# phantomzone-org/fhe-ram

Hardware: AMD Instinct MI355X
Metric: encrypted RAM read ops/s + write ops/s at 2^18 entries; achieved HBM GB/s vs peak (higher is better)
Workload: dtype f64

## Files before the change

fhe-ram_amd/csrc/bank.hpp:

```cpp
#pragma once
#include "path.hpp"

struct fheram_bank {
    fheram_ctx* c = nullptr;
    int M = 0, mws = 0;
    RamState ram[FHERAM_BANK_MAX];
    double* d_prep = nullptr;
    double* d_prep_inv = nullptr;
    ReadBufs list;
    int list_n = 0;
};

namespace {

RamView bank_view(const fheram_bank* b, int first) {
    RamView v = ctx_view(b->c);
    const size_t o1 = (size_t)first * b->mws * fheram_ctx::GLWE, oR = o1 * b->c->rows;
    for (int32_t** p : {&v.rows, &v.A, &v.B, &v.C, &v.D}) *p += oR;
    for (int32_t** p : {&v.part, &v.tmp, &v.tmp2, &v.res, &v.tree, &v.w, &v.trtop}) *p += o1;
    return v;
}
Opnds bank_opnds(fheram_bank* b, RamState* st, const fheram_addr* const* addrs, int n) {
    if (n == 1) return one_addr(b->c, addrs, b->mws, st);
    return table_opnds(b->c, st, addrs, n, b->mws, b->d_prep, b->d_prep_inv, SRC_MAP_IDENTITY, true);
// ... 127 lines not shown
    return FHERAM_OK;
}
void fheram_bank_destroy(fheram_bank* b) {
    if (!b) return;
    if (b->c) {
        hipSetDevice(b->c->device);
        if (b->c->stream) hipStreamSynchronize(b->c->stream);
        if (b->c->stream2) hipStreamSynchronize(b->c->stream2);
    }
    if (b->d_prep) hipFree(b->d_prep);
    if (b->d_prep_inv) hipFree(b->d_prep_inv);
    reads_free(b->list);
    fheram_ctx_destroy(b->c);
    delete b;
}
const char* fheram_bank_last_error(const fheram_bank* b) { return fheram_last_error(b ? b->c : nullptr); }
int fheram_bank_size(const fheram_bank* b) { return b ? b->M : 0; }

int fheram_bank_keys_load(fheram_bank* b, const int64_t* gal_els, int n_gal, const int64_t* const* atk_glwe,
                          const int64_t* atk_ggsw_inv, int64_t atk_ggsw_inv_p, const int64_t* tsk) {
    if (!b) return FHERAM_ERR_INVALID_ARG;
    const int rc = fheram_keys_load(b->c, gal_els, n_gal, atk_glwe, atk_ggsw_inv, atk_ggsw_inv_p, tsk);
    if (rc != FHERAM_OK) return rc;
    for (int m = 0; m < b->M; m++) { b->ram[m].memo_top = false; b->ram[m].memo_alone = 0; }
    return FHERAM_OK;
}
int fheram_bank_ram_upload(fheram_bank* b, int member, const int64_t* rows) {
    if (!b) return FHERAM_ERR_INVALID_ARG;
    fheram_ctx* c = b->c;
    if (member < 0 || member >= b->M) return fail(c, FHERAM_ERR_INVALID_ARG, "no such member");
    if (!rows) return fail(c, FHERAM_ERR_INVALID_ARG, "null rows");
    HIPCHK(c, hipSetDevice(c->device));
    const size_t n = (size_t)b->mws * c->rows * fheram_ctx::GLWE;
    const int rc = upload_i64(c, c->d_data + (size_t)member * n, rows, n);
    if (rc != FHERAM_OK) return rc;
    RamState& r = b->ram[member];
    r.initialized = true; r.state = false; r.memo_top = false; r.memo_alone = 0;
    return FHERAM_OK;
}
int fheram_bank_ram_download(fheram_bank* b, int member, int64_t* rows) {
    if (!b) return FHERAM_ERR_INVALID_ARG;
    fheram_ctx* c = b->c;
    if (member < 0 || member >= b->M || !rows) return fail(c, FHERAM_ERR_INVALID_ARG, "no such member, or null rows");
    if (!b->ram[member].initialized) return fail(c, FHERAM_ERR_UNINITIALIZED, "unitialized memory: self.data.len()=0");
    HIPCHK(c, hipSetDevice(c->device));
    const size_t n = (size_t)b->mws * c->rows * fheram_ctx::GLWE;
    const int rc = download_i64(c, rows, c->d_data + (size_t)member * n, n);
    return rc == FHERAM_OK ? check_precision(c) : rc;
}
int fheram_bank_ram_tree_download(fheram_bank* b, int member, int level, int64_t* out) {
    if (!b) return FHERAM_ERR_INVALID_ARG;
    fheram_ctx* c = b->c;
    if (member < 0 || member >= b->M || !out) return fail(c, FHERAM_ERR_INVALID_ARG, "no such member, or null output");
    if (level != 0 || c->n2 < 2) return fail(c, FHERAM_ERR_INVALID_ARG, "tree level does not exist (ram.rs:315-324)");
    HIPCHK(c, hipSetDevice(c->device));
    const size_t n = (size_t)b->mws * fheram_ctx::GLWE;
    return download_i64(c, out, c->d_tree + (size_t)member * n, n);
}
int fheram_bank_ram_state(const fheram_bank* b, int member) { return (b && member >= 0 && member < b->M) ? (int)b->ram[member].state : 0; }

int fheram_bank_address_create(fheram_bank* b, const int64_t* const* ggsw, int n_ggsw, fheram_addr** out) {
    if (!b) return FHERAM_ERR_INVALID_ARG;
    return fheram_address_create(b->c, ggsw, n_ggsw, out);
}

int fheram_bank_fheuint_create(fheram_bank* b, const int64_t* bits, int n_bits, fheram_fheuint** out) {
// ... 104 lines not shown
```

fhe-ram_amd/csrc/ctx.hpp:

```cpp
#pragma once
#include "../../include/fheram.h"
#include "kernels.hpp"
#include "cmux_chain.hpp"

#include <algorithm>
#include <atomic>
#include <cstdio>
#include <cstdlib>
#include <cstring>
#include <map>
#include <string>
#include <vector>

using namespace fk;

namespace {

thread_local std::string g_create_err;


struct ProfCls {
    uint64_t launches = 0, blocks = 0;
    double ms = 0.0;
    std::vector<std::pair<hipEvent_t, hipEvent_t>> pending;
};

}

inline uint64_t next_addr_id() { static std::atomic<uint64_t> n{0}; return ++n; }

struct RamState {
    bool initialized = false, state = false;
    bool memo_top = false;
    int memo_alone = 0;
    bool res_in_trtop = false;
};

struct ReadBufs {
    int cap = 0;
    int32_t *A = nullptr, *B = nullptr;
    int32_t* C = nullptr;
    int32_t *res = nullptr, *tmp = nullptr, *tmp2 = nullptr;
    double* prep = nullptr;
    int64_t *h_res = nullptr, *d_h_res = nullptr;
};

struct fheram_ctx {
    fheram_params p;
    int device = 0;
    hipStream_t stream = nullptr;
    hipStream_t stream2 = nullptr;
    hipStream_t cur = nullptr;
    hipEvent_t ev_fork = nullptr, ev_join = nullptr;
    hipEvent_t ev_xout = nullptr, ev_xin = nullptr;
    bool side_begun = false;
    bool trhi_in_C = false;
    bool tree_rotate_pending = false;
    int ws = 0, n2 = 0, n_digits = 0;
    size_t rows = 0;
    size_t rows_glob = 0;
    int shard = 0, n_shards = 1;
    std::vector<std::vector<int>> base2d;
    static constexpr int S_CT = 3, S_ADDR = 4, S_INV = 5, DNUM_CT = 3, DNUM_GGSW = 4;
    int s_evk = 4;
    size_t atk = 0;
    static constexpr size_t GLWE = (size_t)S_CT * 2 * N;
    static constexpr size_t GLWE4 = (size_t)S_ADDR * 2 * N;
    static constexpr size_t GGSW = (size_t)DNUM_CT * 2 * GLWE4;
    static constexpr size_t EVK5 = (size_t)DNUM_GGSW * S_INV * 2 * N;
    static constexpr size_t GGSW5 = (size_t)DNUM_GGSW * 2 * S_INV * 2 * N;
    double* d_tw = nullptr;
    double ninv = 0.0;
    double* d_atk = nullptr;
    double* d_atk_inv = nullptr;
    double* d_tsk = nullptr;
    int64_t gal[LOGN];
    bool keys_loaded = false;
    int32_t* d_data = nullptr;
    int32_t* d_tree = nullptr;
    int32_t* d_scrA = nullptr;
    int32_t* d_scrB = nullptr;
    int32_t* d_scrC = nullptr;
    int32_t* d_scrD = nullptr;
    int32_t* d_res = nullptr;
    int32_t* d_tmp = nullptr;
    int32_t* d_tmp2 = nullptr;
    int32_t* d_w = nullptr;
    double* d_big = nullptr;
    double* d_big2 = nullptr;
    int limb_split = 1;
// ... 233 lines not shown
```

fhe-ram_amd/csrc/fheram.hip:

```cpp
#include <unistd.h>
#include <atomic>
#include "path.hpp"

extern "C" {

int fheram_params_default(fheram_params* p) {
    if (!p) return FHERAM_ERR_INVALID_ARG;
    std::memset(p, 0, sizeof(*p));
    p->log_n = 12; p->base2k = 17; p->rank = 1;
    p->k_glwe_pt = 3; p->k_glwe_ct = 51; p->k_ggsw_addr = 68; p->k_evk_trace = 68; p->k_evk_ggsw_inv = 85;
    p->word_size = 4; p->n_decomp = 4;
    p->decomp_n[0] = p->decomp_n[1] = p->decomp_n[2] = p->decomp_n[3] = 3;
    p->max_addr = (uint64_t)1 << 14;
    return FHERAM_OK;
}

const char* fheram_last_error(const fheram_ctx* c) { return c ? c->err.c_str() : g_create_err.c_str(); }

void fheram_config_default(fheram_config* cfg) {
    if (!cfg) return;
    fheram_config d{};
    d.limb_split = 1; d.fine_split = 1; d.memo = 1; d.pre_inv = 1; d.tail = 1; d.tail_test = 0; d.mid = 2; d.mid_test = 0;
    d.chain = 1; d.chain_y = 3; d.pair_z = 1; d.fuse = 1; d.graph = 0; d.safe = 0; d.nco = 0; d.tail_ep = 1; d.monitor = 1; d.reserved = 0;
    auto env = [](const char* n) { const char* v = getenv(n); return (v && v[0]) ? v[0] : '\0'; };
// ... 71 lines not shown
        while (bits != 0) {
            std::vector<int> v;
            for (uint32_t i = 0; i < p->n_decomp; i++) {
                const uint32_t b = p->decomp_n[i];
                if (b <= bits) { v.push_back((int)b); bits -= b; }
                else { if (bits != 0) { v.push_back((int)bits); bits = 0; } break; }
            }
            c->base2d.push_back(v);
        }
    }
    c->n2 = (int)c->base2d.size();
    for (auto& v : c->base2d) { c->n_digits += (int)v.size(); c->max_digits = std::max(c->max_digits, (int)v.size()); }
    for (int i = 0; i < LOGN; i++) c->gal[i] = galois_element(i);

#define CCHK(call)                                                                  \
    do {                                                                            \
        hipError_t e_ = (call);                                                     \
        if (e_ != hipSuccess) {                                                     \
            g_create_err = std::string(#call) + ": " + hipGetErrorString(e_);       \
            fheram_ctx_destroy(c);                                                  \
            return FHERAM_ERR_DEVICE;                                               \
        }                                                                           \
    } while (0)
    CCHK(hipSetDevice(device));
    CCHK(hipStreamCreateWithFlags(&c->stream, hipStreamNonBlocking));
    {
        int lo = 0, hi = 0;
        CCHK(hipDeviceGetStreamPriorityRange(&lo, &hi));
        CCHK(hipStreamCreateWithPriority(&c->stream2, hipStreamNonBlocking, lo));
    }
    c->cur = c->stream;
    CCHK(hipEventCreateWithFlags(&c->ev_fork, hipEventDisableTiming));
    CCHK(hipEventCreateWithFlags(&c->ev_join, hipEventDisableTiming));
    CCHK(hipEventCreateWithFlags(&c->ev_xout, hipEventDisableTiming));
    CCHK(hipEventCreateWithFlags(&c->ev_xin, hipEventDisableTiming));
    CCHK(hipEventCreate(&c->t0));
    CCHK(hipEventCreate(&c->t1));
    {
        fheram_config cfg;
        if (user_cfg) cfg = *user_cfg; else fheram_config_default(&cfg);
        c->limb_split = cfg.limb_split ? 1 : 0;
        c->fine_split = cfg.fine_split ? 1 : 0;
        c->memo = cfg.memo ? 1 : 0;
        c->pre_inv = c->memo ? (cfg.pre_inv == 2 ? 2 : (cfg.pre_inv ? 1 : 0)) : 0;
        c->tail = cfg.tail ? 1 : 0;
        static std::atomic<int> serial{0};
        c->tail_xoff = ((serial++ + (int)getpid()) & 1) * (TAIL_GROUPS / 2);
        c->tail_test = cfg.tail_test < 0 ? 0 : (cfg.tail_test > 2 ? 2 : cfg.tail_test);
        c->tail_ep = cfg.tail_ep ? 1 : 0;
        c->mid = cfg.mid < 0 ? 0 : (cfg.mid > 2 ? 2 : cfg.mid);
        c->mid_test = cfg.mid_test ? 1 : 0;
        c->chain = cfg.chain ? 1 : 0;
        c->chain_y = cfg.chain_y ? 3 : 0;
        c->pair_z = cfg.pair_z ? 1 : 0;
        c->fuse = cfg.fuse ? 1 : 0;
        c->use_graph = cfg.graph ? 1 : 0;
        if (c->use_graph) c->pre_inv = 0;
        c->safe = cfg.safe ? 1 : 0;
        if (c->safe) { c->tail = 0; c->tail_test = 0; c->mid = 0; c->mid_test = 0; if (c->pre_inv == 1) c->pre_inv = 2; }
        c->monitor = cfg.monitor < 0 ? 0 : (cfg.monitor > 2 ? 2 : cfg.monitor);
        if (c->safe && c->monitor == 1) c->monitor = 2;
        c->nco = cfg.nco == 2 ? 2 : (cfg.nco == 1 ? 1 : 0);
        hipDeviceProp_t prop;
        if (hipGetDeviceProperties(&prop, device) == hipSuccess && prop.multiProcessorCount > 0) c->cus = prop.multiProcessorCount;
    }
#define LDSATTR(k) CCHK(hipFuncSetAttribute(reinterpret_cast<const void*>(k), hipFuncAttributeMaxDynamicSharedMemorySize, (int)LDS_BYTES))
    LDSATTR(k_prepare);
    LDSATTR((&k_ext_product<3, 4, 1>));
    LDSATTR((&k_ext_product<3, 4, 2>));
    LDSATTR((&k_ext_product<3, 4, 1, 1>));
    LDSATTR((&k_ext_product_fine<3, 4>));
    LDSATTR((&k_ext_product_fine<4, 5>));
    LDSATTR((&k_ext_product_chain<3, 4>));
    LDSATTR((&k_ext_product_chain_r<4>));
    LDSATTR((&k_pair_z<4>)); LDSATTR((&k_pair_z<5>));
    LDSATTR((&k_read_chain<4, 4>)); LDSATTR((&k_read_chain<5, 4>)); LDSATTR((&k_write_chain<4, 4>)); LDSATTR((&k_write_chain<5, 4>));
    LDSATTR((&k_write_chain_t<4, 4>)); LDSATTR((&k_write_chain_t<5, 4>));
    LDSATTR((&k_read_chain_w<4, 4>)); LDSATTR((&k_read_chain_w<5, 4>));
    LDSATTR((&k_read_chain_t<4, 4>)); LDSATTR((&k_read_chain_t<5, 4>));
    LDSATTR((&k_trace_tail_t<3, 4, 3>)); LDSATTR((&k_trace_tail_t<3, 5, 3>));
    LDSATTR((&k_keyswitch_chain_w<3, 4, 3, 3>)); LDSATTR((&k_keyswitch_chain_w<3, 5, 3, 3>));
    LDSATTR((&k_keyswitch_chain<3, 4, 3>));
    LDSATTR((&k_keyswitch_chain<3, 4, 3, 3>));
    LDSATTR((&k_keyswitch_chain<3, 5, 3, 3>));
    LDSATTR((&k_trace_tail<3, 4, 3>));
    LDSATTR((&k_chain_mid<false, 4, 3, 2>)); LDSATTR((&k_chain_mid<false, 5, 3, 2>)); LDSATTR((&k_chain_mid<true, 4, 3, 2>));
    LDSATTR((&k_chain_mid<false, 4, 1, 1>)); LDSATTR((&k_chain_mid<false, 5, 1, 1>));
    LDSATTR((&k_chain_mid<false, 4, 1, 2>)); LDSATTR((&k_chain_mid<false, 5, 1, 2>));
#define LDSATTR_KS4(M, SX, SK, SO) LDSATTR((&k_keyswitch<M, SX, SK, SO, 1>)); LDSATTR((&k_keyswitch<M, SX, SK, SO, 1, 1>)); LDSATTR((&k_keyswitch_fine<M, SX, SK>))
#define LDSATTR_KS(M, SX, SK, SO) LDSATTR_KS4(M, SX, SK, SO); LDSATTR((&k_keyswitch<M, SX, SK, SO, 2>))
    LDSATTR_KS(KS_AUTO, 3, 4, 3);
    LDSATTR_KS(KS_TRACE, 3, 4, 3);
    LDSATTR_KS4(KS_PAIR, 3, 4, 3);
    LDSATTR_KS(KS_ADD, 3, 4, 3);
    LDSATTR_KS(KS_SUBNEG, 3, 4, 3);
// ... 54 lines not shown
    for (int i = 0; i < 2; i++) CCHK(hipEventCreateWithFlags(&c->ev_inv[i], hipEventDisableTiming));
    CCHK(hipEventCreateWithFlags(&c->ev_wdone, hipEventDisableTiming));
    CCHK(hipEventCreateWithFlags(&c->ev_opstart, hipEventDisableTiming));
    CCHK(hipMalloc(&c->d_tail_sync, (size_t)(TAIL_GROUPS + 1) * 32 * sizeof(unsigned)));
    CCHK(hipMemset(c->d_tail_sync, 0, (size_t)(TAIL_GROUPS + 1) * 32 * sizeof(unsigned)));
    for (int i = 0; i < 2; i++) {
        CCHK(hipMalloc(&c->d_mid_sync[i], (size_t)(MID_GROUPS_MAX + 1) * 32 * sizeof(unsigned)));
        CCHK(hipMemset(c->d_mid_sync[i], 0, (size_t)(MID_GROUPS_MAX + 1) * 32 * sizeof(unsigned)));
        CCHK(hipMalloc(&c->d_mid_y[i], (size_t)2 * MID_GROUPS_MAX * 2 * N * sizeof(double)));
        CCHK(hipMalloc(&c->d_mid_big[i], (size_t)2 * MID_GROUPS_MAX * BIG_STRIDE * sizeof(double)));
    }
    CCHK(hipHostMalloc((void**)&c->h_tail_fb, 64, hipHostMallocDefault));
    *c->h_tail_fb = 0;
    CCHK(hipHostMalloc((void**)&c->h_mid_fb, 128, hipHostMallocDefault));
    memset(c->h_mid_fb, 0, 128);
    CCHK(hipHostMalloc((void**)&c->h_res, ((size_t)c->ws * G + 1) * sizeof(int64_t), hipHostMallocMapped));
    CCHK(hipHostGetDevicePointer((void**)&c->d_h_res, c->h_res, 0));
    CCHK(hipHostMalloc((void**)&c->h_w, (size_t)c->ws * G * sizeof(int32_t), hipHostMallocDefault));
    CCHK(hipEventCreateWithFlags(&c->ev_w, hipEventDisableTiming));
#undef CCHK
    *out = c;
    return FHERAM_OK;
}

void fheram_ctx_destroy(fheram_ctx* c) {
    if (!c) return;
    hipSetDevice(c->device);
    if (c->stream) hipStreamSynchronize(c->stream);
    if (c->stream2) hipStreamSynchronize(c->stream2);
    prof_collect(c);
    reads_free(c->batch);
    if (c->ev_fork) hipEventDestroy(c->ev_fork);
    if (c->ev_join) hipEventDestroy(c->ev_join);
    for (int i = 0; i < 2; i++) if (c->ev_inv[i]) hipEventDestroy(c->ev_inv[i]);
    if (c->ev_wdone) hipEventDestroy(c->ev_wdone);
    if (c->ev_opstart) hipEventDestroy(c->ev_opstart);
    if (c->ev_xout) hipEventDestroy(c->ev_xout);
    if (c->ev_xin) hipEventDestroy(c->ev_xin);
    if (c->stream2) hipStreamDestroy(c->stream2);
    for (auto e : c->ev_pool) hipEventDestroy(e);
    if (c->t0) hipEventDestroy(c->t0);
    if (c->t1) hipEventDestroy(c->t1);
    for (int b = 0; b < 2; b++) { if (c->ev_pin[b]) hipEventDestroy(c->ev_pin[b]); if (c->h_pin[b]) hipHostFree(c->h_pin[b]); }
    void* bufs[] = {c->d_tw, c->d_atk, c->d_atk_inv, c->d_tsk, c->d_data, c->d_scrA, c->d_scrB, c->d_big, c->d_big2, c->d_scrC, c->d_scrD, c->d_ggsw_tmp2, c->d_tmp2, c->d_part, c->d_gat[0], c->d_gat[1], c->d_gat[2], c->d_tree, c->d_res, c->d_tmp, c->d_w, c->d_trtop, c->d_prep, c->d_ggsw_tmp, c->d_tail_sync, c->d_prep_inv, c->d_ggsw_inv, c->d_mid_sync[0], c->d_mid_sync[1], c->d_mid_y[0], c->d_mid_y[1], c->d_mid_big[0], c->d_mid_big[1]};
    for (void* b : bufs) if (b) hipFree(b);
    if (c->h_tail_fb) hipHostFree(c->h_tail_fb);
    if (c->h_mid_fb) hipHostFree(c->h_mid_fb);
    if (c->h_res) hipHostFree(c->h_res);
    if (c->h_ro_flag) hipHostFree(c->h_ro_flag);
    if (c->h_w) hipHostFree(c->h_w);
    if (c->ev_w) hipEventDestroy(c->ev_w);
    if (c->stream) hipStreamDestroy(c->stream);
    delete c;
}

int fheram_ctx_config(const fheram_ctx* c, fheram_config* out) {
    if (!c || !out) return FHERAM_ERR_INVALID_ARG;
    fheram_config d{};
    d.limb_split = c->limb_split; d.fine_split = c->fine_split; d.memo = c->memo; d.pre_inv = c->pre_inv; d.tail = c->tail; d.tail_test = c->tail_test;
    d.mid = c->mid; d.mid_test = c->mid_test; d.chain = c->chain; d.chain_y = c->chain_y; d.pair_z = c->pair_z; d.fuse = c->fuse;
    d.graph = c->use_graph; d.safe = c->safe; d.nco = c->nco; d.monitor = c->monitor; d.tail_ep = c->tail_ep;
    *out = d;
    return FHERAM_OK;
}

size_t fheram_glwe_len(const fheram_ctx*) { return fheram_ctx::GLWE; }
// ... 9 lines not shown
    if (!c) return FHERAM_ERR_INVALID_ARG;
    if (!gal_els || !atk_glwe || !atk_ggsw_inv || !tsk) return fail(c, FHERAM_ERR_INVALID_ARG, "null key pointer");
    if (n_gal != LOGN) return fail(c, FHERAM_ERR_KEYS, "expected log2(N) trace keys (keys.rs:39)");
    if (atk_ggsw_inv_p != -1) return fail(c, FHERAM_ERR_KEYS, "auto_key.p() != -1 (coordinate_prepared.rs:134)");
    HIPCHK(c, hipSetDevice(c->device));
    HIPCHK(c, hipStreamSynchronize(c->stream));
    HIPCHK(c, hipStreamSynchronize(c->stream2));
    int order[LOGN];
    for (int i = 0; i < LOGN; i++) {
        order[i] = -1;
        for (int j = 0; j < n_gal; j++) if (gal_els[j] == c->gal[i]) order[i] = j;
        if (order[i] < 0) return fail(c, FHERAM_ERR_KEYS, "missing trace key for a Galois element of GLWE::trace_galois_elements");
    }
    int32_t* d_stage = nullptr;
    const size_t stage_n = std::max(c->atk, fheram_ctx::EVK5);
    HIPCHK(c, hipMalloc(&d_stage, stage_n * sizeof(int32_t)));
    int rc = FHERAM_OK;
    for (int i = 0; i < LOGN && rc == FHERAM_OK; i++) {
        rc = upload_i64(c, d_stage, atk_glwe[order[i]], c->atk);
        if (rc == FHERAM_OK) launch_prepare(c, d_stage, c->d_atk + (size_t)i * c->atk, (int)(c->atk / N), c->gal[i]);
        hipStreamSynchronize(c->stream);
    }
    if (rc == FHERAM_OK) rc = upload_i64(c, d_stage, atk_ggsw_inv, fheram_ctx::EVK5);
    if (rc == FHERAM_OK) { launch_prepare(c, d_stage, c->d_atk_inv, (int)(fheram_ctx::EVK5 / N), -1); hipStreamSynchronize(c->stream); }
    if (rc == FHERAM_OK) rc = upload_i64(c, d_stage, tsk, fheram_ctx::EVK5);
    if (rc == FHERAM_OK) { launch_prepare(c, d_stage, c->d_tsk, (int)(fheram_ctx::EVK5 / N)); hipStreamSynchronize(c->stream); }
    hipFree(d_stage);
    if (rc != FHERAM_OK) return rc;
    HIPCHK(c, hipGetLastError());
    c->keys_loaded = true;
    c->inv_id[0] = c->inv_id[1] = 0;
    c->inv_pending[0] = c->inv_pending[1] = false;
    c->ram.memo_top = false; c->ram.memo_alone = 0;
    return FHERAM_OK;
}

int fheram_ram_upload(fheram_ctx* c, const int64_t* rows) {
    if (!c) return FHERAM_ERR_INVALID_ARG;
    if (!rows) return fail(c, FHERAM_ERR_INVALID_ARG, "null rows");
    HIPCHK(c, hipSetDevice(c->device));
    int rc = upload_i64(c, c->d_data, rows, (size_t)c->ws * c->rows * fheram_ctx::GLWE);
    if (rc != FHERAM_OK) return rc;
    c->ram.initialized = true; c->ram.state = false; c->ram.memo_top = false; c->ram.memo_alone = 0;
    return FHERAM_OK;
}
int fheram_ram_download(fheram_ctx* c, int64_t* rows) {
    if (!c || !rows) return FHERAM_ERR_INVALID_ARG;
    if (!c->ram.initialized) return fail(c, FHERAM_ERR_UNINITIALIZED, "unitialized memory: self.data.len()=0");
    HIPCHK(c, hipSetDevice(c->device));
    const int rc = download_i64(c, rows, c->d_data, (size_t)c->ws * c->rows * fheram_ctx::GLWE);
    return rc == FHERAM_OK ? check_precision(c) : rc;
}
int fheram_ram_tree_download(fheram_ctx* c, int level, int64_t* out) {
    if (!c || !out) return FHERAM_ERR_INVALID_ARG;
    if (level != 0 || c->n2 < 2) return fail(c, FHERAM_ERR_INVALID_ARG, "tree level does not exist (ram.rs:315-324)");
    HIPCHK(c, hipSetDevice(c->device));
    return download_i64(c, out, c->d_tree, (size_t)c->ws * fheram_ctx::GLWE);
}
int fheram_ram_state(const fheram_ctx* c) { return c ? (int)c->ram.state : 0; }

int fheram_address_create(fheram_ctx* c, const int64_t* const* ggsw, int n_ggsw, fheram_addr** out) {
    if (!c || !out) return FHERAM_ERR_INVALID_ARG;
    *out = nullptr;
    if (!ggsw) return fail(c, FHERAM_ERR_INVALID_ARG, "null ggsw");
    if (n_ggsw != c->n_digits) return fail(c, FHERAM_ERR_INVALID_ARG, "address digit count does not match the context's Base2D (ram.rs:404)");
    HIPCHK(c, hipSetDevice(c->device));
    fheram_addr* a = new fheram_addr{c, nullptr, n_ggsw, c->device};
    hipError_t e = hipMalloc(&a->d_ggsw, (size_t)n_ggsw * fheram_ctx::GGSW * sizeof(int32_t));
    if (e != hipSuccess) { delete a; return fail(c, FHERAM_ERR_DEVICE, std::string("hipMalloc: ") + hipGetErrorString(e)); }
    for (int i = 0; i < n_ggsw; i++) {
        if (!ggsw[i]) { fheram_address_destroy(a); return fail(c, FHERAM_ERR_INVALID_ARG, "null ggsw digit"); }
        int rc = upload_i64(c, a->d_ggsw + (size_t)i * fheram_ctx::GGSW, ggsw[i], fheram_ctx::GGSW);
        if (rc != FHERAM_OK) { fheram_address_destroy(a); return rc; }
// ... 498 lines not shown
```

fhe-ram_amd/csrc/path.hpp:

```cpp
#pragma once
#include "launch.hpp"

namespace {

struct Opnds {
    fheram_ctx* c;
    RamState* st;
    const fheram_addr* const* addrs;
    int n, ws;
    double *tab, *tab_inv;
    long stride;
    unsigned src_map;
    bool bank;
    int member(int k) const { return (int)((src_map >> (4 * k)) & 15u); }
    int Y() const { return n * ws; }
    double* prep(int k, int ci) const { return digits_of(c, tab + k * stride, ci); }
    double* inv(int k, int ci) const { return digits_of(c, tab_inv + k * stride, ci); }
    GlweRef slice(GlweRef r, int k) const { r.p += (long)k * ws * r.sy; return r; }
    GlweRef rows(GlweRef r, int k) const { return slice(r, member(k)); }
    OpndTable table() const { return n == 1 ? OpndTable{} : OpndTable{ws, stride, src_map}; }
    bool row_fuse(int d, int n_tr, int gx) const { return use_row_fuse(c, d, n_tr, gx, Y(), bank); }
};
Opnds one_addr(fheram_ctx* c, const fheram_addr* const* a, int ws, RamState* st) { return Opnds{c, st, a, 1, ws, c->d_prep, c->d_prep_inv, 0, 0, false}; }
Opnds one_addr(fheram_ctx* c, const fheram_addr* const* a) { return one_addr(c, a, c->ws, &c->ram); }
Opnds table_opnds(fheram_ctx* c, RamState* st, const fheram_addr* const* addrs, int n, int ws, double* tab, double* tab_inv, unsigned src_map, bool bank) {
    return Opnds{c, st, addrs, n, ws, tab, tab_inv, (long)c->n_digits * (long)fheram_ctx::GGSW, src_map, bank};
}

struct RamView {
    int32_t *rows, *A, *B, *C, *D;
    int32_t *part, *tmp, *tmp2, *res, *tree, *w, *trtop;
};
RamView ctx_view(const fheram_ctx* c) {
    return RamView{c->d_data, c->d_scrA, c->d_scrB, c->d_scrC, c->d_scrD, c->d_part, c->d_tmp, c->d_tmp2, c->d_res, c->d_tree, c->d_w, c->d_trtop};
}

void read_local_done(const fheram_ctx* c, RamState* st, bool prepare_write) {
    if (c->n2 == 2) st->memo_alone = (prepare_write && c->memo) ? LOGN - ilog2_ceil(c->rows_glob) : 0;
}
void read_top_done(fheram_ctx* c, RamState* st, bool prepare_write) {
    st->memo_top = prepare_write && c->memo;
    st->res_in_trtop = st->memo_top;
    c->prep1_ready = false;
}
void write_done(fheram_ctx* c, RamState* st) { st->memo_top = false; st->memo_alone = 0; c->side_begun = false; c->tree_rotate_pending = false; }

template <typename F>
int run_op(fheram_ctx* c, const fheram_addr* addr, int which, F&& enqueue) {
    if (!c->use_graph || c->profile) return enqueue();
    fheram_addr* a = const_cast<fheram_addr*>(addr);
    const unsigned sig = 1u | (c->ram.memo_top ? 2u : 0u) | ((unsigned)c->ram.memo_alone << 2) | (c->side_begun ? 64u : 0u) |
                         (c->inv_id[0] == addr->id ? 128u : 0u) | (c->inv_id[1] == addr->id ? 256u : 0u);
    if (a->graph[which] && a->graph_sig[which] != sig) { hipGraphExecDestroy(a->graph[which]); a->graph[which] = nullptr; }
    if (!a->graph[which]) {
        hipGraph_t g = nullptr;
        HIPCHK(c, hipStreamBeginCapture(c->stream, hipStreamCaptureModeThreadLocal));
        const int rc = enqueue();
        const hipError_t e = hipStreamEndCapture(c->stream, &g);
        if (rc != FHERAM_OK || e != hipSuccess) {
            if (g) hipGraphDestroy(g);
            return rc != FHERAM_OK ? rc : fail(c, FHERAM_ERR_DEVICE, std::string("hipStreamEndCapture: ") + hipGetErrorString(e));
        }
        const hipError_t e2 = hipGraphInstantiate(&a->graph[which], g, nullptr, nullptr, 0);
        hipGraphDestroy(g);
        if (e2 != hipSuccess) { a->graph[which] = nullptr; return fail(c, FHERAM_ERR_DEVICE, std::string("hipGraphInstantiate: ") + hipGetErrorString(e2)); }
        a->graph_sig[which] = sig;
    }
    HIPCHK(c, hipGraphLaunch(a->graph[which], c->stream));
    if (which == 2) write_done(c, &c->ram);
    else { read_local_done(c, &c->ram, which == 1); read_top_done(c, &c->ram, which == 1); }
    return FHERAM_OK;
}

int check_common(fheram_ctx* c, const fheram_addr* addr) {
    if (!c) return FHERAM_ERR_INVALID_ARG;
    mid_rearm(c);
    if (!addr || addr->ctx != c) return fail(c, FHERAM_ERR_INVALID_ARG, "address does not belong to this context (layout mismatch, ram.rs:404)");
    if (addr->empty) return fail(c, FHERAM_ERR_INVALID_ARG, "empty address: fheram_address_alloc without fheram_address_derive");
    if (!c->ram.initialized) return fail(c, FHERAM_ERR_UNINITIALIZED, "unitialized memory: self.data.len()=0");
    if (!c->keys_loaded) return fail(c, FHERAM_ERR_KEYS, "evaluation keys not loaded");
    return FHERAM_OK;
}

int read_local(const Opnds& o, const RamView& a, bool prepare_write, GlweRef* packed_out, bool to_part) {
    fheram_ctx* c = o.c;
    const int n = o.n, ws = o.ws, Y = o.Y(), R = (int)c->rows;
    c->wide = !prepare_write || n > 1;
    if (n == 1 && prepare_write && c->pre_inv == 1 && !capturing(c) && (c->wide_unsynced || c->derive_unsynced)) {
        hipEventRecord(c->ev_opstart, c->stream);
        c->opstart_valid = true;
    }
    const long G = (long)fheram_ctx::GLWE;
    const long sy = (long)c->rows * G;
    GlweRef data = ref(a.rows, sy, G), A = ref(a.A, sy, G), B = ref(a.B, sy, G);
    GlweRef part = ref(a.part, G, 0);
    const bool all = (c->n_shards == 1 && c->n2 == 2);
    for (int k = 0; k < n; k++)
        if (all) coordinate_prepare_all(c, o.addrs[k], o.tab + k * o.stride); else coordinate_prepare(c, o.addrs[k], 0, o.tab + k * o.stride);
    c->prep1_ready = all;
    read_local_done(c, o.st, prepare_write);
    const int d0 = (int)c->base2d[0].size();
    if (c->n2 == 1) {
        GlweRef row0 = ref(a.rows, sy, 0);
        for (int k = 0; k < n; k++)
// ... 35 lines not shown
        if (gathered) {
            const int kG = ilog2_ceil((size_t)c->n_shards);
            int32_t* a0 = c->d_gat[1];
            int32_t* a1 = c->d_gat[2];
            int32_t* packed = pack_levels(c, gathered, a0, a1, G, (long)ws * G, (size_t)c->n_shards, ws, 0, LOGN - kG);
            pk = ref(packed, G, 0);
        }
        if (!c->prep1_ready) coordinate_prepare(c, o.addrs[0], 1, o.tab);
        if (!fuse_ep) products1();
        last = ep_out;
    }
    const bool pre = n == 1 && prepare_write && c->pre_inv && (long)c->rows * Y <= c->cus;
    const bool gated = pre && c->pre_inv == 1 && !capturing(c) && tail_top();
    if (pre && !gated)
        for (int ci = c->n2 - 1; ci >= 0; ci--) precompute_inverse(c, o.addrs[0], ci, ci == c->n2 - 1);
    read_top_done(c, o.st, prepare_write);
    const GlweRef res = ref(o.st->memo_top ? a.trtop : a.res, G, 0);
    const uint64_t tl0 = c->tail_launches;
    GlweRef tb[2];
    if (fuse_ep && chain_bufs(LOGN, last, res, tmp, tb))
        launch_trace_tail(c, pk, tb, 0, LOGN, 1, Y, o.prep(0, 1), d1, ep_out, prepare_write, o.table());
    else {
        if (fuse_ep) products1();
        trace_steps(c, last, res, tmp, 0, LOGN, 1, Y);
    }
    if (gated && !c->opstart_valid && (c->wide_unsynced || c->derive_unsynced)) {
        hipEventRecord(c->ev_opstart, c->stream);
        c->opstart_valid = true;
    }
    if (gated) {
        const unsigned seq = c->tail_launches != tl0 ? c->tail_seq : 0;
        for (int ci = c->n2 - 1; ci >= 0; ci--) precompute_inverse(c, o.addrs[0], ci, ci == c->n2 - 1, seq);
    }
    return FHERAM_OK;
}
int read_impl(const Opnds& o, const RamView& a, bool prepare_write) {
    fheram_ctx* c = o.c;
    GlweRef packed;
    int rc = read_local(o, a, prepare_write, &packed, false);
    if (rc != FHERAM_OK) return rc;
    rc = read_top(o, a, prepare_write, nullptr, packed);
    if (o.n == 1 && prepare_write && c->inv_id[0] == o.addrs[0]->id && capturing(c))
        for (int ci = 0; ci < c->n2; ci++) hipStreamWaitEvent(c->stream, c->ev_inv[ci], 0);
    if (rc == FHERAM_OK && prepare_write) o.st->state = true;
    return rc;
}

void reads_free(ReadBufs& L) {
    void* bufs[] = {L.A, L.B, L.C, L.res, L.tmp, L.tmp2, L.prep};
    for (void* p : bufs) if (p) hipFree(p);
    if (L.h_res) hipHostFree(L.h_res);
    L = ReadBufs{};
}
bool third_arena_needed(const fheram_ctx* c, int n_ct) {
    return c->n2 == 2 && chain_form(c, ChainQuery{false, LOGN - ilog2_ceil(c->rows_glob), (int)c->rows, n_ct}).form == ChainForm::Tail;
}
int reads_reserve(fheram_ctx* c, ReadBufs& L, int n, int ws) {
    const bool work = n > 1, third = work && third_arena_needed(c, n * ws);
    if (n <= L.cap && (!work || L.A) && (!third || L.C)) return FHERAM_OK;
    if (n < L.cap) n = L.cap;
    const bool had_work = L.A != nullptr, had_third = L.C != nullptr;
    if (L.cap) { HIPCHK(c, hipStreamSynchronize(c->stream)); reads_free(L); }
    const size_t G = fheram_ctx::GLWE, nct = (size_t)n * ws, nrow = nct * c->rows;
    hipError_t e = hipSuccess;
    auto dev = [&](auto** p, size_t bytes) { if (e == hipSuccess) e = hipMalloc((void**)p, bytes); };
    dev(&L.res, nct * G * sizeof(int32_t));
// ... 55 lines not shown

int write_top(const Opnds& o, const RamView& v) {
    fheram_ctx* c = o.c;
    c->wide = true;
    const long G = (long)fheram_ctx::GLWE;
    const long sy = (long)c->rows * G;
    const int n = o.n, ws = o.ws, Y = o.Y();
    GlweRef wref = ref(v.w, G, 0), tmp = ref(v.tmp, G, 0), tmp2 = ref(v.tmp2, G, 0), tree = ref(v.tree, G, 0);
    GlweRef top = (c->n2 != 1) ? tree : ref(v.rows, sy, 0);
    GlweRef tr = tmp;
    if (o.st->memo_top) tr = ref(v.trtop, G, 0);
    else trace_steps(c, top, tmp, tmp2, 0, LOGN, 1, Y);
    {
        ProfScope ps(c, "elementwise", Y);
        hipLaunchKernelGGL((k_sub_add_norm<3>), dim3(1, Y, EW_SLICES), dim3(256), 0, c->cur, top, tr, wref, top);
    }
    o.st->memo_top = false;
    if (c->n2 == 2) {
        if (n == 1 && c->inv_id[1] == o.addrs[0]->id) wait_inverse(c, c->stream, 1);
        else {
            if (n == 1 && c->inv_pending[1]) wait_inverse(c, c->stream, 1);
            for (int k = 0; k < n; k++) coordinate_prepare_inv(c, o.addrs[k], 1, c->d_ggsw_tmp, o.inv(k, 1));
        }
        if (n == 1) { c->inv_pending[1] = false; c->inv_id[1] = 0; }
        for (int k = 0; k < n; k++)
            ep_chain(c, o.slice(tree, k), o.slice(ref(v.part, G, 0), k), o.slice(tmp, k), o.inv(k, 1), (int)c->base2d[1].size(), 1, ws);
        c->tree_rotate_pending = true;
    }
    return FHERAM_OK;
}
void write_side_begin(const Opnds& o, const RamView& v) {
    fheram_ctx* c = o.c;
    c->wide = true;
    const long G = (long)fheram_ctx::GLWE;
    const long sy = (long)c->rows * G;
    hipEventRecord(c->ev_fork, c->stream);
    hipStreamWaitEvent(c->stream2, c->ev_fork, 0);
    c->cur = c->stream2;
    if (c->n2 == 2) {
        const int kept = o.st->memo_alone;
        c->trhi_in_C = kept > 0 && (LOGN - kept) % 2 == 1;
        if (kept > 0) trace_steps(c, ref(v.A, sy, G), ref(c->trhi_in_C ? v.C : v.A, sy, G), ref(c->trhi_in_C ? v.A : v.C, sy, G), kept, LOGN, (int)c->rows, o.Y());
        else trace_steps(c, ref(v.rows, sy, G), ref(v.A, sy, G), ref(v.C, sy, G), 0, LOGN, (int)c->rows, o.Y());
        o.st->memo_alone = 0;
    }
    if (o.n == 1 && c->inv_id[0] == o.addrs[0]->id) wait_inverse(c, c->stream2, 0);
    else for (int k = 0; k < o.n; k++) coordinate_prepare_inv(c, o.addrs[k], 0, c->d_ggsw_tmp2, o.inv(k, 0));
    if (o.n == 1) { c->inv_id[0] = 0; c->inv_pending[0] = false; }
    hipEventRecord(c->ev_join, c->stream2);
    c->cur = c->stream;
    c->side_begun = true;
}
void write_side_abort(fheram_ctx* c) {
    if (!c->side_begun) return;
    hipStreamWaitEvent(c->stream, c->ev_join, 0);
    c->side_begun = false;
}
int write_rows(const Opnds& o, const RamView& v) {
    fheram_ctx* c = o.c;
    c->wide = true;
    const long G = (long)fheram_ctx::GLWE;
    const long sy = (long)c->rows * G;
    const int n = o.n, ws = o.ws, Y = o.Y(), R = (int)c->rows;
    GlweRef data = ref(v.rows, sy, G), A = ref(v.A, sy, G), B = ref(v.B, sy, G), D = ref(v.D, sy, G);
    GlweRef trhi = ref(c->trhi_in_C ? v.C : v.A, sy, G), part = ref(v.part, G, 0);
    const int d0 = (int)c->base2d[0].size();
    const bool fuse = c->n2 == 2 && o.row_fuse(d0, LOGN, R);
    if (fuse) {
        hipStreamWaitEvent(c->stream, c->ev_join, 0);
        launch_write_chain(c, part, c->n_shards, c->shard, data, trhi, o.inv(0, 0), d0, LOGN, R, Y, o.table());
    } else if (c->n2 == 2)
        trace_steps(c, part, B, D, 0, LOGN, R, Y, c->n_shards, c->shard);
    if (c->tree_rotate_pending) {
        ProfScope ps(c, "elementwise", Y);
        hipLaunchKernelGGL((k_rotate<3>), dim3(1, Y, EW_SLICES), dim3(256), 0, c->cur, part, ref(v.tree, G, 0), -(int)c->rows_glob);
    }
    if (!fuse) {
        hipStreamWaitEvent(c->stream, c->ev_join, 0);
// ... 14 lines not shown
```

fhe-ram_amd/csrc/setup.hpp:

```cpp
#pragma once
#include "launch.hpp"

namespace {
void wipe_free(hipStream_t st, void* d, size_t bytes) {
    if (!d) return;
    if (hipMemsetAsync(d, 0, bytes, st) == hipSuccess) hipStreamSynchronize(st);
    hipFree(d);
}
void wipe_host(void* p, size_t bytes) {
    volatile unsigned char* v = static_cast<volatile unsigned char*>(p);
    for (size_t i = 0; i < bytes; i++) v[i] = 0;
}
}

namespace {

constexpr int64_t NOISE_LIM = (int64_t)1 << 30;
int noise_limb(int k) { return (k + BASE2K - 1) / BASE2K - 1; }

template <int S, int DEC>
void launch_enc(fheram_ctx* c, int32_t* cts, const double* s_hat, const int32_t* pt1, int n) {
    ProfScope ps(c, "encrypt", (uint64_t)n);
    hipLaunchKernelGGL((k_encrypt_sk<S, DEC>), dim3(n), dim3(T), LDS_BYTES, c->cur, cts, s_hat, c->d_tw, pt1);
}
// ... 160 lines not shown
    const size_t ws = (size_t)c->ws;
    if (data_len % ws != 0) return fail(c, FHERAM_ERR_INVALID_ARG, "invalid data: data.len()%ram_chunks != 0");
    if (data_len / ws != c->p.max_addr) return fail(c, FHERAM_ERR_INVALID_ARG, "invalid data: data.len()/ram_chunks != max_addr");
    const int k = (int)c->p.k_glwe_ct, S = fheram_ctx::S_CT;
    int rc = check_setup_args(c, sk, S, k);
    if (rc != FHERAM_OK) return rc;
    const int k_pt = (int)c->p.k_glwe_pt, size_pt = (k_pt + BASE2K - 1) / BASE2K;
    if (k_pt <= 0 || k_pt > 8 + BASE2K || size_pt > S) return fail(c, FHERAM_ERR_UNSUPPORTED, "k_glwe_pt out of range");
    HIPCHK(c, hipSetDevice(c->device));
    const size_t G = fheram_ctx::GLWE, max_addr = c->p.max_addr;
    const size_t CH = 256;
    std::vector<int32_t> pre(std::min(CH, c->rows) * G);
    int32_t limbs[4];
    for (size_t w = 0; w < ws; w++)
        for (size_t x0 = 0; x0 < c->rows; x0 += CH) {
            const size_t nx = std::min(CH, c->rows - x0);
            std::fill(pre.begin(), pre.begin() + nx * G, 0);
            for (size_t x = 0; x < nx; x++) {
                const size_t r = (size_t)c->shard + (x0 + x) * (size_t)c->n_shards;
                int32_t* pg = pre.data() + x * G;
                for (size_t q = 0; q < (size_t)N; q++) {
                    const size_t a = r * N + q;
                    if (a >= max_addr) break;
                    encode_value((int64_t)(int8_t)data[a * ws + w], k_pt, size_pt, limbs);
                    for (int j = 0; j < size_pt; j++) pg[(size_t)(j * 2) * N + q] = limbs[j];
                }
                const size_t gi = w * c->rows + x0 + x;
                if (!stage_random(pg, S, k, mask + gi * S * N, noise + gi * N))
                    return fail(c, FHERAM_ERR_RANGE, "mask limb outside [-2^16, 2^16) or |noise| >= 2^30");
            }
            rc = encrypt_staged(c, sk->d_hat, c->d_data + (w * c->rows + x0) * G, pre, nullptr, (int)nx, S);
            if (rc != FHERAM_OK) return rc;
        }
    c->ram.initialized = true; c->ram.state = false;
    return FHERAM_OK;
}

int fheram_address_encrypt_sk(fheram_ctx* c, const fheram_secret* sk, uint32_t value, const int64_t* mask,
                              const int64_t* noise, fheram_addr** out) {
    if (!c || !out) return FHERAM_ERR_INVALID_ARG;
    *out = nullptr;
    if (!mask || !noise) return fail(c, FHERAM_ERR_INVALID_ARG, "null argument");
    const int S = fheram_ctx::S_ADDR, k = (int)c->p.k_ggsw_addr, D = fheram_ctx::DNUM_CT;
    int rc = check_setup_args(c, sk, S, k);
    if (rc != FHERAM_OK) return rc;
    HIPCHK(c, hipSetDevice(c->device));
    {
        unsigned bits = 0;
        for (auto& b1 : c->base2d) for (int b : b1) bits += (unsigned)b;
        if (bits < 32 && ((uint64_t)value >> bits) != 0)
            return fail(c, FHERAM_ERR_INVALID_ARG, "self.base2d.max() > value (address.rs:98): address does not fit the digit plan");
    }
    const size_t glen = fheram_ctx::GLWE4;
    const int n = c->n_digits * D * 2;
    std::vector<int32_t> pre((size_t)n * glen, 0), pt1((size_t)n * S * N, 0);
    size_t remain = value;
    int gi = 0;
    for (auto& base1d : c->base2d) {
        unsigned tot = 0;
        for (int b : base1d) tot += (unsigned)b;
        const size_t max = (size_t)1 << tot;
        size_t rem_c = remain & (max - 1);
        remain /= max;
        const bool neg = rem_c != 0;
        unsigned tot_base = 0;
        for (int b : base1d) {
// ... 64 lines not shown
    auto automorphism_key = [&](int64_t p, int rows, int S, int k, double* d_prepared, int64_t* std_dst) -> int {
        host_automorphism(galois_inv_mod(galois_mod(p)), sk->sk.data(), sk_out.data());
        hipMemcpyAsync(d_small, sk_out.data(), N * sizeof(int32_t), hipMemcpyHostToDevice, c->stream);
        launch_prepare(c, d_small, d_hat, 1);
        hipStreamSynchronize(c->stream);
        return gglwe(sk->sk.data(), d_hat, rows, S, k, d_prepared, std_dst, p);
    };
    for (int i = 0; i < LOGN && rc == FHERAM_OK; i++)
        rc = automorphism_key(c->gal[i], fheram_ctx::DNUM_CT, c->s_evk, (int)c->p.k_evk_trace,
                              c->d_atk + (size_t)i * c->atk, std_out ? std_out + (size_t)i * c->atk : nullptr);
    if (rc == FHERAM_OK) {
        std::copy(sk->sk.begin(), sk->sk.end(), ss.begin() + N);
        hipMemcpyAsync(d_small, ss.data(), 2 * N * sizeof(int32_t), hipMemcpyHostToDevice, c->stream);
        launch_enc_dyn(c, 1, 1, d_small, sk->d_hat, nullptr, 1);
        hipMemcpyAsync(ss.data(), d_small, N * sizeof(int32_t), hipMemcpyDeviceToHost, c->stream);
        if (hipStreamSynchronize(c->stream) != hipSuccess) rc = fail(c, FHERAM_ERR_DEVICE, "tensor key: s*s failed");
    }
    if (rc == FHERAM_OK)
        rc = gglwe(ss.data(), sk->d_hat, fheram_ctx::DNUM_GGSW, fheram_ctx::S_INV, (int)c->p.k_evk_ggsw_inv, c->d_tsk,
                   std_out ? std_out + (size_t)LOGN * c->atk : nullptr, 0);
    if (rc == FHERAM_OK)
        rc = automorphism_key(-1, fheram_ctx::DNUM_GGSW, fheram_ctx::S_INV, (int)c->p.k_evk_ggsw_inv, c->d_atk_inv,
                              std_out ? std_out + (size_t)LOGN * c->atk + fheram_ctx::EVK5 : nullptr);
    hipFree(d_stage);
    wipe_free(c->stream, d_small, 2 * N * sizeof(int32_t));
    wipe_free(c->stream, d_hat, N * sizeof(double));
    wipe_host(sk_out.data(), sk_out.size() * sizeof(sk_out[0])); wipe_host(ss.data(), ss.size() * sizeof(ss[0]));
    if (rc != FHERAM_OK) return rc;
    HIPCHK(c, hipGetLastError());
    c->keys_loaded = true;
    c->inv_id[0] = c->inv_id[1] = 0;
    c->inv_pending[0] = c->inv_pending[1] = false;
    c->ram.memo_top = false; c->ram.memo_alone = 0;
    return FHERAM_OK;
}

size_t fheram_fheuint_ggsw_len(const fheram_ctx*) { return fheram_ctx::GGSW5; }
namespace {
int fheuint_alloc(fheram_ctx* c, int n_bits, fheram_fheuint** out) {
    fheram_fheuint* f = new fheram_fheuint{c, c->device, n_bits, nullptr, nullptr};
    hipError_t e = hipMalloc(&f->d_std, (size_t)n_bits * fheram_ctx::GGSW5 * sizeof(int32_t));
    if (e == hipSuccess) e = hipMalloc(&f->d_prep, (size_t)n_bits * fheram_ctx::GGSW5 * sizeof(double));
    if (e != hipSuccess) { fheram_fheuint_destroy(f); return fail(c, FHERAM_ERR_DEVICE, std::string("hipMalloc: ") + hipGetErrorString(e)); }
    *out = f;
    return FHERAM_OK;
}
int fheuint_prepare(fheram_ctx* c, fheram_fheuint* f) {
    c->cur = c->stream;
    launch_prepare(c, f->d_std, f->d_prep, f->n_bits * (int)(fheram_ctx::GGSW5 / N));
    HIPCHK(c, hipStreamSynchronize(c->stream));
    HIPCHK(c, hipGetLastError());
    return FHERAM_OK;
}
}
int fheram_fheuint_create(fheram_ctx* c, const int64_t* bits, int n_bits, fheram_fheuint** out) {
    if (!c || !out) return FHERAM_ERR_INVALID_ARG;
    *out = nullptr;
    if (!bits || n_bits <= 0 || n_bits > 64) return fail(c, FHERAM_ERR_INVALID_ARG, "bad argument");
    HIPCHK(c, hipSetDevice(c->device));
    fheram_fheuint* f = nullptr;
    int rc = fheuint_alloc(c, n_bits, &f);
    if (rc == FHERAM_OK) rc = upload_i64(c, f->d_std, bits, (size_t)n_bits * fheram_ctx::GGSW5);
    if (rc == FHERAM_OK) rc = fheuint_prepare(c, f);
    if (rc != FHERAM_OK) { fheram_fheuint_destroy(f); return rc; }
    *out = f;
    return FHERAM_OK;
// ... 170 lines not shown
```

Before: 1305.

## Start high-level trace steps early on side stream after read prep

Result: no change. 1316, median of 6 (+0.8%).

```diff
diff --git a/fhe-ram_amd/csrc/bank.hpp b/fhe-ram_amd/csrc/bank.hpp
--- a/fhe-ram_amd/csrc/bank.hpp
+++ b/fhe-ram_amd/csrc/bank.hpp
@@ -183,6 +183,7 @@
     if (!rows) return fail(c, FHERAM_ERR_INVALID_ARG, "null rows");
     HIPCHK(c, hipSetDevice(c->device));
     const size_t n = (size_t)b->mws * c->rows * fheram_ctx::GLWE;
+    trace_hi_void(c);
     const int rc = upload_i64(c, c->d_data + (size_t)member * n, rows, n);
     if (rc != FHERAM_OK) return rc;
     RamState& r = b->ram[member];
diff --git a/fhe-ram_amd/csrc/ctx.hpp b/fhe-ram_amd/csrc/ctx.hpp
--- a/fhe-ram_amd/csrc/ctx.hpp
+++ b/fhe-ram_amd/csrc/ctx.hpp
@@ -56,6 +56,10 @@
     bool side_begun = false;
     bool trhi_in_C = false;
     bool tree_rotate_pending = false;
+    bool trhi_begun = false;
+    const int32_t* trhi_arena = nullptr;
+    hipEvent_t ev_opend = nullptr, ev_trhi = nullptr;
+    int pre_trace = 1;
     int ws = 0, n2 = 0, n_digits = 0;
     size_t rows = 0;
     size_t rows_glob = 0;
diff --git a/fhe-ram_amd/csrc/fheram.hip b/fhe-ram_amd/csrc/fheram.hip
--- a/fhe-ram_amd/csrc/fheram.hip
+++ b/fhe-ram_amd/csrc/fheram.hip
@@ -127,6 +127,8 @@
     c->cur = c->stream;
     CCHK(hipEventCreateWithFlags(&c->ev_fork, hipEventDisableTiming));
     CCHK(hipEventCreateWithFlags(&c->ev_join, hipEventDisableTiming));
+    CCHK(hipEventCreateWithFlags(&c->ev_opend, hipEventDisableTiming));
+    CCHK(hipEventCreateWithFlags(&c->ev_trhi, hipEventDisableTiming));
     CCHK(hipEventCreateWithFlags(&c->ev_xout, hipEventDisableTiming));
     CCHK(hipEventCreateWithFlags(&c->ev_xin, hipEventDisableTiming));
     CCHK(hipEventCreate(&c->t0));
@@ -156,6 +158,7 @@
         c->monitor = cfg.monitor < 0 ? 0 : (cfg.monitor > 2 ? 2 : cfg.monitor);
         if (c->safe && c->monitor == 1) c->monitor = 2;
         c->nco = cfg.nco == 2 ? 2 : (cfg.nco == 1 ? 1 : 0);
+        if (const char* v = getenv("FHERAM_PRE_TRACE")) c->pre_trace = v[0] == '0' ? 0 : 1;
         hipDeviceProp_t prop;
         if (hipGetDeviceProperties(&prop, device) == hipSuccess && prop.multiProcessorCount > 0) c->cus = prop.multiProcessorCount;
     }
@@ -276,6 +279,8 @@
     reads_free(c->batch);
     if (c->ev_fork) hipEventDestroy(c->ev_fork);
     if (c->ev_join) hipEventDestroy(c->ev_join);
+    if (c->ev_opend) hipEventDestroy(c->ev_opend);
+    if (c->ev_trhi) hipEventDestroy(c->ev_trhi);
     for (int i = 0; i < 2; i++) if (c->ev_inv[i]) hipEventDestroy(c->ev_inv[i]);
     if (c->ev_wdone) hipEventDestroy(c->ev_wdone);
     if (c->ev_opstart) hipEventDestroy(c->ev_opstart);
@@ -351,6 +356,7 @@
     c->inv_id[0] = c->inv_id[1] = 0;
     c->inv_pending[0] = c->inv_pending[1] = false;
     c->ram.memo_top = false; c->ram.memo_alone = 0;
+    trace_hi_void(c);
     return FHERAM_OK;
 }
 
@@ -358,6 +364,7 @@
     if (!c) return FHERAM_ERR_INVALID_ARG;
     if (!rows) return fail(c, FHERAM_ERR_INVALID_ARG, "null rows");
     HIPCHK(c, hipSetDevice(c->device));
+    trace_hi_void(c);
     int rc = upload_i64(c, c->d_data, rows, (size_t)c->ws * c->rows * fheram_ctx::GLWE);
     if (rc != FHERAM_OK) return rc;
     c->ram.initialized = true; c->ram.state = false; c->ram.memo_top = false; c->ram.memo_alone = 0;
diff --git a/fhe-ram_amd/csrc/path.hpp b/fhe-ram_amd/csrc/path.hpp
--- a/fhe-ram_amd/csrc/path.hpp
+++ b/fhe-ram_amd/csrc/path.hpp
@@ -50,7 +50,8 @@
     if (!c->use_graph || c->profile) return enqueue();
     fheram_addr* a = const_cast<fheram_addr*>(addr);
     const unsigned sig = 1u | (c->ram.memo_top ? 2u : 0u) | ((unsigned)c->ram.memo_alone << 2) | (c->side_begun ? 64u : 0u) |
-                         (c->inv_id[0] == addr->id ? 128u : 0u) | (c->inv_id[1] == addr->id ? 256u : 0u);
+                         (c->inv_id[0] == addr->id ? 128u : 0u) | (c->inv_id[1] == addr->id ? 256u : 0u) |
+                         (c->trhi_begun ? 512u : 0u);
     if (a->graph[which] && a->graph_sig[which] != sig) { hipGraphExecDestroy(a->graph[which]); a->graph[which] = nullptr; }
     if (!a->graph[which]) {
         hipGraph_t g = nullptr;
@@ -70,6 +71,34 @@
     if (which == 2) write_done(c, &c->ram);
     else { read_local_done(c, &c->ram, which == 1); read_top_done(c, &c->ram, which == 1); }
     return FHERAM_OK;
+}
+
+void trace_hi(fheram_ctx* c, RamState* st, const RamView& v, int Y, const char* cls) {
+    const long G = (long)fheram_ctx::GLWE;
+    const long sy = (long)c->rows * G;
+    const int kept = st->memo_alone;
+    ProfScope ps(c, cls, (uint64_t)c->rows * Y, LOGN - kept);
+    c->trhi_in_C = kept > 0 && (LOGN - kept) % 2 == 1;
+    if (kept > 0) trace_steps(c, ref(v.A, sy, G), ref(c->trhi_in_C ? v.C : v.A, sy, G), ref(c->trhi_in_C ? v.A : v.C, sy, G), kept, LOGN, (int)c->rows, Y);
+    else trace_steps(c, ref(v.rows, sy, G), ref(v.A, sy, G), ref(v.C, sy, G), 0, LOGN, (int)c->rows, Y);
+    st->memo_alone = 0;
+}
+void trace_hi_early(const Opnds& o, const RamView& v) {
+    fheram_ctx* c = o.c;
+    hipEventRecord(c->ev_opend, c->stream);
+    hipStreamWaitEvent(c->stream2, c->ev_opend, 0);
+    const bool wide = c->wide;
+    hipStream_t keep = c->cur;
+    c->wide = true; c->cur = c->stream2;
+    trace_hi(c, o.st, v, o.Y(), "trace_hi_early");
+    hipEventRecord(c->ev_trhi, c->stream2);
+    c->cur = keep; c->wide = wide;
+    c->trhi_begun = true; c->trhi_arena = v.A;
+}
+void trace_hi_void(fheram_ctx* c) {
+    if (!c->trhi_begun) return;
+    hipStreamWaitEvent(c->stream, c->ev_trhi, 0);
+    c->trhi_begun = false;
 }
 
 int check_common(fheram_ctx* c, const fheram_addr* addr) {
@@ -171,6 +200,7 @@
         const unsigned seq = c->tail_launches != tl0 ? c->tail_seq : 0;
         for (int ci = c->n2 - 1; ci >= 0; ci--) precompute_inverse(c, o.addrs[0], ci, ci == c->n2 - 1, seq);
     }
+    if (pre && c->pre_trace && c->n_shards == 1 && c->n2 == 2 && o.st->memo_alone > 0 && !capturing(c)) trace_hi_early(o, a);
     return FHERAM_OK;
 }
 int read_impl(const Opnds& o, const RamView& a, bool prepare_write) {
@@ -292,18 +322,12 @@
 void write_side_begin(const Opnds& o, const RamView& v) {
     fheram_ctx* c = o.c;
     c->wide = true;
-    const long G = (long)fheram_ctx::GLWE;
-    const long sy = (long)c->rows * G;
     hipEventRecord(c->ev_fork, c->stream);
     hipStreamWaitEvent(c->stream2, c->ev_fork, 0);
     c->cur = c->stream2;
-    if (c->n2 == 2) {
-        const int kept = o.st->memo_alone;
-        c->trhi_in_C = kept > 0 && (LOGN - kept) % 2 == 1;
-        if (kept > 0) trace_steps(c, ref(v.A, sy, G), ref(c->trhi_in_C ? v.C : v.A, sy, G), ref(c->trhi_in_C ? v.A : v.C, sy, G), kept, LOGN, (int)c->rows, o.Y());
-        else trace_steps(c, ref(v.rows, sy, G), ref(v.A, sy, G), ref(v.C, sy, G), 0, LOGN, (int)c->rows, o.Y());
-        o.st->memo_alone = 0;
-    }
+    const bool early = c->trhi_begun && c->trhi_arena == v.A;
+    c->trhi_begun = false;
+    if (c->n2 == 2 && !early) trace_hi(c, o.st, v, o.Y(), "trace_hi_write");
     if (o.n == 1 && c->inv_id[0] == o.addrs[0]->id) wait_inverse(c, c->stream2, 0);
     else for (int k = 0; k < o.n; k++) coordinate_prepare_inv(c, o.addrs[k], 0, c->d_ggsw_tmp2, o.inv(k, 0));
     if (o.n == 1) { c->inv_id[0] = 0; c->inv_pending[0] = false; }
diff --git a/fhe-ram_amd/csrc/setup.hpp b/fhe-ram_amd/csrc/setup.hpp
--- a/fhe-ram_amd/csrc/setup.hpp
+++ b/fhe-ram_amd/csrc/setup.hpp
@@ -216,6 +216,7 @@
             rc = encrypt_staged(c, sk->d_hat, c->d_data + (w * c->rows + x0) * G, pre, nullptr, (int)nx, S);
             if (rc != FHERAM_OK) return rc;
         }
+    trace_hi_void(c);
     c->ram.initialized = true; c->ram.state = false;
     return FHERAM_OK;
 }
@@ -346,6 +347,7 @@
     c->inv_id[0] = c->inv_id[1] = 0;
     c->inv_pending[0] = c->inv_pending[1] = false;
     c->ram.memo_top = false; c->ram.memo_alone = 0;
+    trace_hi_void(c);
     return FHERAM_OK;
 }
 
```
